# leavesnight/VIEO_SLAM

Measured on AMD Instinct MI355X. Metric: frontend+localBA frames/sec on EuRoC MH05 stereo-VIO; ATE vs ref, higher is better.
Workload: dtype u8 (extract/match) + f64 (pose optimisation)

## Files before the change

### include/vieo_hot.h

```cpp
#ifndef VIEO_HOT_H
#define VIEO_HOT_H

#include <stddef.h>
#include <stdint.h>

#ifdef __cplusplus
extern "C" {
#endif

#define VIEO_OK 0
#define VIEO_E_INVALID (-1)
#define VIEO_E_NO_DEVICE (-2)
#define VIEO_E_HIP (-3)
#define VIEO_E_CAPACITY (-4)
#define VIEO_E_EMPTY (-5)

const char* vieo_last_error(void);
int vieo_device_available(void);
int vieo_set_device(int device);
int vieo_get_device(void);
const char* vieo_version(void);

int vieo_dev_malloc(void** d_ptr, size_t bytes);
int vieo_dev_free(void* d_ptr);
// ... 582 lines not shown
                                            const int32_t* d_cam_first, int n_cams, int key_cap, int n_frames, int img_first,
                                            int img_step, const float* d_inv_sigma2, vieo_pose_obs* d_obs, int32_t* d_obs_key,
                                            void* d_frames, int frames_are_vio, void* stream);
int vieo_track_build_obs_depth_batch_device(const int32_t* d_mp_ref, const float* d_point_xyz,
                                            const float* d_point_depth, float close_depth, int p_cap,
                                            const vieo_keypoint* d_keys, const float* d_uright,
                                            const int32_t* d_counts, int key_cap, int n_frames,
                                            int img_first, int img_step, const float* d_inv_sigma2,
                                            vieo_pose_obs* d_obs, int32_t* d_obs_key, void* d_frames,
                                            int frames_are_vio, void* stream);
int vieo_track_merge_assign_rig_batch_device(const int32_t* d_assign, int32_t* d_mp_ref, const int32_t* d_counts,
                                             int key_cap, int n_frames, int img_first, int img_step, int point_offset,
                                             int reset, int query_div,
                                             const vieo_last_frame_point* d_same_point ,
                                             const int32_t* d_query_src , int q_cap, void* stream);
int vieo_track_compact_queries_batch_device(const vieo_proj_query* d_queries, const int32_t* d_nq, int q_cap, int n_frames,
                                            vieo_proj_query* d_queries_out, int32_t* d_src, int32_t* d_nq_out, void* stream);
int vieo_track_build_obs_rig_batch_device(const int32_t* d_mp_ref, const float* d_point_xyz,
                                          const float* d_point_depth, float close_depth, int p_cap,
                                          const vieo_keypoint* d_keys, const float* d_uright,
                                          const int32_t* d_counts, const int32_t* d_cam_first, int n_cams, int key_cap,
                                          int n_frames, const float* d_inv_sigma2, vieo_pose_obs* d_obs,
                                          int32_t* d_obs_key, void* d_frames, int frames_are_vio, void* stream);
int vieo_track_mark_held_batch_device(const int32_t* d_mp_ref, const int32_t* d_counts, int key_cap,
                                      int n_frames, int img_first, int img_step, uint8_t* d_held, int p_cap,
                                      void* stream);
void* vieo_orb_stream(vieo_orb* e);

int vieo_orb_tap_plane(vieo_orb* e, int image_index, int level, int which, uint8_t* h_dst,
                       int dst_stride);
int vieo_orb_tap_candidates(vieo_orb* e, int image_index, int level, int32_t* h_dst, int cap);
int vieo_orb_tap_level_keys(vieo_orb* e, int image_index, int level, vieo_keypoint* h_dst,
                            int cap);


typedef struct vieo_frustum_frame {
  float Rcrw[9], tcrw[3];
  float Ow[3];
  int32_t n_cams;
  int32_t use_distort;
  const struct vieo_camera* cams;
  float Tcr[4][12];
  float trc[4][3];
  float bounds[4][4];
  float bf;
  float log_scale_factor;
  int32_t n_levels;
  float viewing_cos_limit;
} vieo_frustum_frame;

typedef struct vieo_frustum_point {
  float Xw[3], normal[3];
  float max_distance, min_distance;
} vieo_frustum_point;

typedef struct vieo_track_info {
  float u[4], v[4], ur[4], viewcos[4];
  int32_t level[4], cam[4];
  int32_t n;
  float track_depth;
} vieo_track_info;

int vieo_is_in_frustum_batch(const vieo_frustum_frame* h_frame, const vieo_frustum_point* h_points, int n_points,
                             vieo_track_info* h_info);
int vieo_track_local_queries_device(const vieo_frustum_frame* h_frame, const vieo_vio_frame* d_frame,
                                    const vieo_vio_result* d_result, const vieo_frustum_point* d_points,
// ... 220 lines not shown
```

### vieo_slam_amd/_lib.py

```python
import ctypes
import os

_HERE = os.path.dirname(os.path.abspath(__file__))
LIB_PATH = os.environ.get("VIEO_LIB_PATH") or os.path.join(_HERE, "libvieo_hot.so")

VIEO_OK = 0
VIEO_E_INVALID, VIEO_E_NO_DEVICE, VIEO_E_HIP, VIEO_E_CAPACITY, VIEO_E_EMPTY = -1, -2, -3, -4, -5

c_p = ctypes.c_void_p
c_i = ctypes.c_int
c_f = ctypes.c_float
c_sz = ctypes.c_size_t
P = ctypes.POINTER

_SIGS = {
    "vieo_last_error": (ctypes.c_char_p, []),
    "vieo_device_available": (c_i, []),
    "vieo_set_device": (c_i, [c_i]),
    "vieo_pose_set_camera_mode": (c_i, [c_i]),
    "vieo_pose_set_replicas": (c_i, [c_i]),
    "vieo_search_for_triangulation": (c_i, [c_p, c_p, c_i, c_i, c_i, c_i, c_i, c_p, c_p, c_p]),
    "vieo_pose_set_encoder_mode": (c_i, [c_i]),
    "vieo_triangulate_new_points": (c_i, [c_p, c_p, c_p, c_p, c_i, c_f, c_i, c_i, c_p, c_p, c_p, c_p, c_p, c_p]),
    "vieo_create_new_map_points": (c_i, [c_p, c_p, c_p, c_p, c_i, c_i, c_i, c_f, c_i, c_i, c_p, c_p, c_p, c_p, c_p, c_p, c_p]),
# ... 101 lines not shown
                                                       c_p, c_i, c_p]),
    "vieo_track_mark_held_batch_device": (c_i, [c_p, c_p, c_i, c_i, c_i, c_i, c_p, c_i, c_p]),
    "vieo_track_after_pose_held_batch_device": (c_i, [c_p, c_p, c_p, c_p, c_p, c_i, c_i, c_i, c_p, c_p, c_p, c_i, c_i, c_p, c_i, c_p]),
    "vieo_track_merge_build_obs_batch_device": (c_i, [c_p, c_p, c_i, c_i, c_i, c_p, c_p, c_i, c_p, c_p, c_f, c_i, c_p, c_p, c_p, c_p, c_i,
                                                       c_i, c_i, c_i, c_i, c_p, c_p, c_p, c_p, c_i, c_p]),
    "vieo_track_local_queries_device": (c_i, [c_p, c_p, c_p, c_p, c_p, c_p, c_p, c_i, c_i, c_f, c_f, c_p, c_p, c_p, c_p, c_p]),
    "vieo_orb_stream": (c_p, [c_p]),
    "vieo_local_bundle_adjustment": (c_i, [c_p, c_p, c_i, c_p, c_i, c_p, c_i, c_p, c_p, c_p, c_p, c_p]),
    "vieo_local_bundle_adjustment_batch": (c_i, [c_i, c_p, c_p, c_p, c_p, c_p, c_p, c_p, c_p, c_p, c_p, c_p,
                                                  c_p]),
    "vieo_local_bundle_adjustment_vio": (c_i, [c_p, c_p, c_i, c_p, c_p, c_i, c_p, c_i, c_p, c_i, c_p, c_p, c_p,
                                                c_p, c_p]),
    "vieo_local_bundle_adjustment_vio_batch": (c_i, [c_i] + [c_p] * 15),
    "vieo_lba_sharded_buffer_doubles": (ctypes.c_size_t, [c_i, c_p]),
    "vieo_lba_enable_timing": (None, [c_i]),
    "vieo_lba_set_stream_priority": (c_i, [c_i]),
    "vieo_lba_kernel_classes": (c_i, []),
    "vieo_lba_kernel_class_name": (ctypes.c_char_p, [c_i]),
    "vieo_lba_kernel_times": (None, [c_p, c_p, c_p]),
    "vieo_lba_sparse_stats": (None, [c_p]),
    "vieo_rccl_available": (c_i, []),
    "vieo_rccl_unique_id": (c_i, [c_p]),
    "vieo_rccl_comm_create": (c_i, [P(c_p), c_p, c_i, c_i]),
    "vieo_rccl_comm_destroy": (c_i, [c_p]),
    "vieo_global_bundle_adjustment_vio_sharded": (c_i, [c_p, c_i, c_i, c_p, c_i, c_p, c_i, c_p, c_i, c_p, c_i, c_p,
                                                        ctypes.c_size_t, c_p, c_p, c_p, c_p, c_p]),
    "vieo_local_bundle_adjustment_vio_sharded": (c_i, [c_i] + [c_p] * 10 + [c_p, ctypes.c_size_t, c_p, c_p] +
                                                 [c_p] * 4),
    "vieo_local_bundle_adjustment_vio_sharded_stop": (c_i, [c_i] + [c_p] * 10 + [c_p, ctypes.c_size_t, c_p, c_p, c_p] +
                                                      [c_p] * 4),
    "vieo_orb_tap_plane": (c_i, [c_p, c_i, c_i, c_i, c_p, c_i]),
    "vieo_orb_tap_candidates": (c_i, [c_p, c_i, c_i, c_p, c_i]),
    "vieo_orb_tap_level_keys": (c_i, [c_p, c_i, c_i, c_p, c_i]),
    "vieo_imu_preintegrate_batch_device": (c_i, [c_p] * 7 + [c_i] + [c_p] * 4),
    "vieo_imu_preintegrate_batch_device_ex": (c_i, [c_p] * 7 + [c_i] + [c_p] * 7),
    "vieo_tracker_create": (c_i, [P(c_p), c_p]),
    "vieo_tracker_create_rig": (c_i, [P(c_p), c_p, c_p]),
    "vieo_tracker_key_capacity": (c_i, [c_p]),
    "vieo_tracker_group_capacity": (c_i, [c_p]),
    "vieo_tracker_image_buffer": (c_i, [c_p, c_i, P(c_p)]),
    "vieo_tracker_destroy": (None, [c_p]),
    "vieo_tracker_image_buffers": (c_i, [c_p, P(c_p), P(c_p)]),
    "vieo_tracker_scale_factors": (c_i, [c_p, c_p]),
    "vieo_track_frame": (c_i, [c_p, c_p, c_p]),
    "vieo_tracker_get_stats": (c_i, [c_p, c_p]),
    "vieo_tracker_reprobe": (c_i, [c_p]),
    "vieo_tracker_get_level": (c_i, [c_p, c_i, c_i, c_i, c_p, c_i]),
    "vieo_tracker_multi_create": (c_i, [P(c_p), c_p, c_i]),
    "vieo_tracker_multi_destroy": (None, [c_p]),
    "vieo_tracker_multi_image_buffer": (c_i, [c_p, c_i, c_i, P(c_p)]),
    "vieo_tracker_multi_reset_slot": (c_i, [c_p, c_i]),
    "vieo_track_frames": (c_i, [c_p, c_i, c_p, c_p, c_p]),
    "vieo_track_local_queries_slot_batch_device": (c_i, [c_p, c_p, c_sz, c_p, c_sz, c_i, c_p, c_p, c_p, c_p, c_p, c_i, c_p, c_i,
                                                         c_f, c_f, c_p, c_p, c_p, c_sz, c_p, c_p]),
}

_lib = None


class VieoError(RuntimeError):
    pass


def declared_symbols():
    return sorted(_SIGS)

# ... 55 lines not shown
```

### vieo_slam_amd/csrc/orb_extractor.hip

```cpp
#include <algorithm>
#include <cmath>
#include <type_traits>
#include <vector>

#include "../../include/vieo_orb_pattern_31.h"
#include "common.h"
#include "sincosf_exact.h"
#include "wave_ops.h"

#define QT_DEVICE
#include "quadtree.inl"

#include "orb_internal.h"

namespace vieo {

#ifndef VIEO_RESIZE_ROWS
#define VIEO_RESIZE_ROWS 32
#endif
static const int kResizeRows = VIEO_RESIZE_ROWS;
#ifndef VIEO_QT_GROUPS
#define VIEO_QT_GROUPS {1, 64}
#endif

// ... 690 lines not shown
    const unsigned oe = ((e[0] >> 16) & 0xFFu) | (((e[1] >> 16) & 0xFFu) << 8) | (((e[2] >> 16) & 0xFFu) << 16) |
                        (((e[3] >> 16) & 0xFFu) << 24);
    const unsigned oo = ((o[0] >> 16) & 0xFFu) | (((o[1] >> 16) & 0xFFu) << 8) | (((o[2] >> 16) & 0xFFu) << 16) |
                        (((o[3] >> 16) & 0xFFu) << 24);
    *(unsigned*)(dst + (size_t)gy * D.pitch + gx) = oe;
    if (gy + 1 < D.h) *(unsigned*)(dst + (size_t)(gy + 1) * D.pitch + gx) = oo;
  }
}

__device__ __forceinline__ int wave_sum(int v) { return wave_sum_i32(v); }

__device__ __forceinline__ float fast_atan2_deg(float y, float x) {
  const float p1 = 0.9997878412794807f * (float)(180 / 3.1415926535897932384626433832795);
  const float p3 = -0.3258083974640975f * (float)(180 / 3.1415926535897932384626433832795);
  const float p5 = 0.1555786518463281f * (float)(180 / 3.1415926535897932384626433832795);
  const float p7 = -0.04432655554792128f * (float)(180 / 3.1415926535897932384626433832795);
  const float eps = (float)2.2204460492503131e-16;
  const float ax = fabsf(x), ay = fabsf(y);
  float a, c, c2;
  if (ax >= ay) {
    c = ay / (ax + eps);
    c2 = c * c;
    a = (((p7 * c2 + p5) * c2 + p3) * c2 + p1) * c;
  } else {
    c = ax / (ay + eps);
    c2 = c * c;
    a = 90.f - (((p7 * c2 + p5) * c2 + p3) * c2 + p1) * c;
  }
  if (x < 0) a = 180.f - a;
  if (y < 0) a = 360.f - a;
  return a;
}

__global__ void __launch_bounds__(256)
k_desc_index(OrbParams P, const unsigned* __restrict__ sel, const int* __restrict__ sel_count,
             uint2* __restrict__ krec, int out_cap, int* __restrict__ counts) {
  const int b = blockIdx.y, g = blockIdx.x * 256 + threadIdx.x;
  int level = -1, idx = 0, total = 0;
  for (int l = 0; l < P.nlevels; l++) {
    const int n = max(sel_count[b * kMaxLevels + l], 0);
    if (level < 0 && g < total + n) {
      level = l;
      idx = g - total;
    }
    total += n;
  }
  if (g == 0) {
    counts[2 * b] = min(total, out_cap);
    counts[2 * b + 1] = 0;
  }
  if (g >= P.kp_cap) return;
  unsigned key = 0;
  if (level >= 0) key = sel[(size_t)b * P.sel_per_image + P.lv[level].sel_off + idx];
  krec[(size_t)b * P.kp_cap + g] = make_uint2(key, (unsigned)level);
}

#ifndef VIEO_DESC_KPW
#define VIEO_DESC_KPW 1
#endif
__global__ void __launch_bounds__(256)
k_describe(OrbParams P, ImgSet I, const uint2* __restrict__ krec, const int* __restrict__ pattern,
           vieo_keypoint* __restrict__ kp_out, uint8_t* __restrict__ desc_out, int out_cap,
           int groups_per_image, int n_images) {
  constexpr int KPW = VIEO_DESC_KPW;
  const int item = xcd_grouped(blockIdx.x, groups_per_image);
  const int b = item / groups_per_image;
  if (b >= n_images) return;
  const int lane = threadIdx.x & 63;
  const int wv = __builtin_amdgcn_readfirstlane((int)(threadIdx.x >> 6));
  const int g0 = ((item - b * groups_per_image) * (blockDim.x >> 6) + wv) * KPW;
  const int gmax = min(P.kp_cap, out_cap);
  if (g0 >= gmax) return;
  uint2 kr[KPW];
#pragma unroll
  for (int u = 0; u < KPW; u++) kr[u] = g0 + u < gmax ? krec[(size_t)b * P.kp_cap + g0 + u] : make_uint2(0, 0xFFFFFFFFu);
  constexpr int AP = 40, BR = 19, BP = 44;
  __shared__ __attribute__((aligned(16))) uint8_t s_patch[4][KPW][31 * AP + (2 * BR + 1) * BP];
  int pt4[4];
#pragma unroll
  for (int gq = 0; gq < 4; gq++) pt4[gq] = pattern[gq * 64 + lane];
  int cxs[KPW], cys[KPW], xas[KPW], xbs[KPW];
  unsigned va[KPW][8], vb[KPW][10];
  const int c = lane & 15, r0 = lane >> 4;
#pragma unroll
  for (int u = 0; u < KPW; u++) {
    const int level = (int)kr[u].y;
    if (level < 0) continue;
    const unsigned key = kr[u].x;
    const LevelDesc& D = P.lv[level];
    const int cx = QT_KEY_X(key) + (kEdge - 3), cy = QT_KEY_Y(key) + (kEdge - 3);
    int pitch;
    const uint8_t* img = plane_ptr(P, I, b, level, &pitch);
    const int xa = (cx - kHalfPatch) & ~3, xb = (cx - BR) & ~3;
    cxs[u] = cx, cys[u] = cy, xas[u] = xa, xbs[u] = xb;
    const uint8_t* bl0 = I.blur + (size_t)b * I.blur_img + D.boff;
    const int bp = D.pitch;
    const uint8_t* ga = img + (size_t)(cy - kHalfPatch + r0) * pitch + xa + 4 * c;
    const uint8_t* gb = bl0 + (size_t)(cy - BR + r0) * bp + xb + 4 * c;
#pragma unroll
    for (int k = 0; k < 8; k++)
      if (c < 9 && r0 + 4 * k < 31) va[u][k] = *(const unsigned*)(ga + (size_t)(4 * k) * pitch);
#pragma unroll
    for (int k = 0; k < 10; k++)
      if (c < 11 && r0 + 4 * k < 2 * BR + 1) vb[u][k] = *(const unsigned*)(gb + (size_t)(4 * k) * bp);
  }
#pragma unroll
  for (int u = 0; u < KPW; u++) {
    if ((int)kr[u].y < 0) continue;
// ... 42 lines not shown
    const float factorPI = (float)(3.1415926535897932384626433832795 / 180.f);
    float a, bsin;
    vieo_sincosf_exact(angle * factorPI, &bsin, &a);
    const uint8_t* bl = sb + BR * BP + (cx - xb);
    unsigned long long bits[4];
#pragma unroll
    for (int gq = 0; gq < 4; gq++) {
      const int pt = pt4[gq];
      const float x0 = (float)(signed char)(pt & 0xFF), y0 = (float)(signed char)((pt >> 8) & 0xFF);
      const float x1 = (float)(signed char)((pt >> 16) & 0xFF), y1 = (float)(signed char)((pt >> 24) & 0xFF);
      const int t0 = bl[__float2int_rn(x0 * bsin + y0 * a) * BP + __float2int_rn(x0 * a - y0 * bsin)];
      const int t1 = bl[__float2int_rn(x1 * bsin + y1 * a) * BP + __float2int_rn(x1 * a - y1 * bsin)];
      bits[gq] = __ballot(t0 < t1);
    }
    if (lane < 4) ((unsigned long long*)(desc_out + ((size_t)b * out_cap + g) * 32))[lane] = bits[lane];
    if (lane == 0) {
      vieo_keypoint k;
      const float fx = (float)cx, fy = (float)cy;
      k.x = level ? fx * D.scale : fx;
      k.y = level ? fy * D.scale : fy;
      k.size = (float)D.patch;
      k.angle = angle;
      k.response = (float)QT_KEY_R(key);
      k.octave = level;
      k.class_id = -1;
      kp_out[(size_t)b * out_cap + g] = k;
    }
  }
}

#ifndef VIEO_FUSED_AB
#define VIEO_FUSED_AB 0
#endif
constexpr int kFR = 18, kFRaw = kFR + 3;
constexpr int kFRawRows = 2 * kFRaw + 1, kFRawPitch = 48;
constexpr int kFHPairs = (kFRawRows + 1) / 2, kFHCols = 40;
constexpr int kFBlRows = 2 * kFR + 1, kFBlPitch = 40;
constexpr int kFWaveLds = kFRawRows * kFRawPitch + 16 + kFHPairs * kFHCols * 4;
static_assert(kFBlRows * kFBlPitch <= kFRawRows * kFRawPitch, "the blurred patch fits where the raw one was");

#ifndef VIEO_FUSED_KPW
#define VIEO_FUSED_KPW 4
#endif
static inline int fused_kpw(int n_images) { return n_images >= 32 ? VIEO_FUSED_KPW : 1; }
__global__ void __launch_bounds__(256)
k_describe_fused(OrbParams P, ImgSet I, const uint2* __restrict__ krec, const int* __restrict__ pattern,
                 vieo_keypoint* __restrict__ kp_out, uint8_t* __restrict__ desc_out, int out_cap,
                 int groups_per_image, int n_images, int KPW) {
  const int item = xcd_grouped(blockIdx.x, groups_per_image);
  const int b = item / groups_per_image;
  if (b >= n_images) return;
  const int lane = threadIdx.x & 63;
  const int wv = __builtin_amdgcn_readfirstlane((int)(threadIdx.x >> 6));
  const int g0 = ((item - b * groups_per_image) * (blockDim.x >> 6) + wv) * KPW;
  const int gmax = min(P.kp_cap, out_cap);
  if (g0 >= gmax) return;
  __shared__ __attribute__((aligned(16))) uint8_t s_all[4][kFWaveLds];
  int pt4[4];
#pragma unroll
  for (int gq = 0; gq < 4; gq++) pt4[gq] = pattern[gq * 64 + lane];
  uint8_t* s_raw = s_all[wv];
  unsigned* s_h = (unsigned*)(s_raw + kFRawRows * kFRawPitch + 16);
  constexpr int NLD = (kFRawRows + 3) / 4;
  unsigned v[NLD];
  bool interior = false;
  int sh = 0;
  const int c = lane & 15, r0 = lane >> 4;
  auto rec_of = [&](int u) { return (u < KPW && g0 + u < gmax) ? krec[(size_t)b * P.kp_cap + g0 + u] : make_uint2(0u, 0xFFFFFFFFu); };
  auto fetch = [&](const uint2 kr) {
    const int level = (int)kr.y;
    if (level < 0) return;
    const LevelDesc& D = P.lv[level];
    const int cx = QT_KEY_X(kr.x) + (kEdge - 3), cy = QT_KEY_Y(kr.x) + (kEdge - 3);
    int pitch;
    const uint8_t* img = plane_ptr(P, I, b, level, &pitch);
    const int x_lo = cx - kFRaw, y_lo = cy - kFRaw;
    const int xa = x_lo & ~3;
    sh = x_lo - xa;
    interior = x_lo >= 0 && y_lo >= 0 && cx + kFRaw < D.w && cy + kFRaw < D.h && xa + 52 <= pitch && ((pitch & 3) == 0) &&
               ((((uintptr_t)img) & 3) == 0);
    if (VIEO_FUSED_AB & 2) {
#pragma unroll
      for (int k = 0; k < NLD; k++) v[k] = kr.x + k;
      interior = false;
    } else if (interior) {
      const uint8_t* gp = img + (size_t)(y_lo + r0) * pitch + xa + 4 * c;
#pragma unroll
      for (int k = 0; k < NLD; k++) {
        v[k] = 0;
        if (c < 13 && r0 + 4 * k < kFRawRows) v[k] = *(const unsigned*)(gp + (size_t)(4 * k) * pitch);
      }
    } else {
#pragma unroll
      for (int k = 0; k < NLD; k++) {
        v[k] = 0;
        if (c < 12 && r0 + 4 * k < kFRawRows) {
          const uint8_t* row = img + (size_t)reflect101(min(max(y_lo + r0 + 4 * k, -(D.h - 1)), 2 * D.h - 2), D.h) * pitch;
#pragma unroll
          for (int jj = 0; jj < 4; jj++) {
            const int x = min(max(x_lo + 4 * c + jj, -(D.w - 1)), 2 * D.w - 2);
            v[k] |= (unsigned)row[reflect101(x, D.w)] << (8 * jj);
          }
        }
      }
    }
  };
  uint2 kr = rec_of(0);
  fetch(kr);
#pragma unroll 1
  for (int u = 0; u < KPW; u++) {
    const uint2 cur = kr;
    const int level = (int)cur.y;
    if (level < 0) break;
    const unsigned key = cur.x;
    const int g = g0 + u;
    const LevelDesc& D = P.lv[level];
    const int cx = QT_KEY_X(key) + (kEdge - 3), cy = QT_KEY_Y(key) + (kEdge - 3);
    if (interior) {
#pragma unroll
      for (int k = 0; k < NLD; k++) {
        const unsigned nxt = (unsigned)__builtin_amdgcn_update_dpp(0, (int)v[k], 0x101, 0xF, 0xF, false);
        v[k] = __builtin_amdgcn_alignbyte(nxt, v[k], sh);
      }
    }
#pragma unroll
    for (int k = 0; k < NLD; k++)
      if (c < 12 && r0 + 4 * k < kFRawRows) *(unsigned*)(s_raw + (r0 + 4 * k) * kFRawPitch + 4 * c) = v[k];
    __builtin_amdgcn_fence(__ATOMIC_ACQ_REL, "workgroup");
    __builtin_amdgcn_wave_barrier();
    kr = rec_of(u + 1);
    fetch(kr);
    {
      constexpr unsigned A0 = 18u | (34u << 8) | (48u << 16) | (56u << 24), A1 = 48u | (34u << 8) | (18u << 16);
      constexpr unsigned B0 = (18u << 8) | (34u << 16) | (48u << 24), B1 = 56u | (48u << 8) | (34u << 16) | (18u << 24);
      constexpr unsigned C0 = (18u << 16) | (34u << 24), C1 = 48u | (56u << 8) | (48u << 16) | (34u << 24), C2 = 18u;
      constexpr unsigned E0 = 18u << 24, E1 = 34u | (48u << 8) | (56u << 16) | (48u << 24), E2 = 34u | (18u << 8);
      for (int idx = lane; idx < ((VIEO_FUSED_AB & 1) ? 0 : kFHPairs * (kFHCols / 8)); idx += 64) {
        const int pr = idx / (kFHCols / 8), g8 = idx - pr * (kFHCols / 8);
        unsigned h[2][8];
#pragma unroll
        for (int q = 0; q < 2; q++) {
          const int r = min(2 * pr + q, kFRawRows - 1);
          const uint2* w = (const uint2*)(s_raw + r * kFRawPitch + 8 * g8);
          const uint2 lo = w[0], hi = w[1];
          const unsigned d0 = lo.x, d1 = lo.y, d2 = hi.x, d3 = hi.y;
#define DOT4(x, k, acc) __builtin_amdgcn_udot4(x, k, acc, false)
          h[q][0] = DOT4(d1, A1, DOT4(d0, A0, 0u));
          h[q][1] = DOT4(d1, B1, DOT4(d0, B0, 0u));
          h[q][2] = DOT4(d2, C2, DOT4(d1, C1, DOT4(d0, C0, 0u)));
          h[q][3] = DOT4(d2, E2, DOT4(d1, E1, DOT4(d0, E0, 0u)));
          h[q][4] = DOT4(d2, A1, DOT4(d1, A0, 0u));
          h[q][5] = DOT4(d2, B1, DOT4(d1, B0, 0u));
          h[q][6] = DOT4(d3, C2, DOT4(d2, C1, DOT4(d1, C0, 0u)));
          h[q][7] = DOT4(d3, E2, DOT4(d2, E1, DOT4(d1, E0, 0u)));
#undef DOT4
        }
        uint4 o0, o1;
        o0.x = h[0][0] | (h[1][0] << 16), o0.y = h[0][1] | (h[1][1] << 16);
        o0.z = h[0][2] | (h[1][2] << 16), o0.w = h[0][3] | (h[1][3] << 16);
        o1.x = h[0][4] | (h[1][4] << 16), o1.y = h[0][5] | (h[1][5] << 16);
        o1.z = h[0][6] | (h[1][6] << 16), o1.w = h[0][7] | (h[1][7] << 16);
        uint4* dst = (uint4*)(s_h + pr * kFHCols + 8 * g8);
        dst[0] = o0, dst[1] = o1;
      }
    }
    int m10 = 0, m01 = 0;
    if (lane < ((VIEO_FUSED_AB & 4) ? 1 : 62)) {
      const int vv = (lane >> 1) - kHalfPatch;
      const int d = P.umax[vv < 0 ? -vv : vv];
      const uint8_t* row = s_raw + (vv + kFRaw) * kFRawPitch + kFRaw;
      const int u0 = (lane & 1) ? 0 : -d, u1 = (lane & 1) ? d : -1;
      int sI = 0;
#pragma unroll
      for (int t = 0; t < 16; t++) {
        const int uu = u0 + t;
        if (uu <= u1) {
          const int val = row[uu];
          m10 += uu * val;
          sI += val;
        }
      }
      m01 = vv * sI;
    }
    m10 = wave_sum(m10);
    m01 = wave_sum(m01);
    const float angle = fast_atan2_deg((float)m01, (float)m10);
    __builtin_amdgcn_fence(__ATOMIC_ACQ_REL, "workgroup");
    __builtin_amdgcn_wave_barrier();
    typedef unsigned short us2 __attribute__((ext_vector_type(2)));
    uint8_t* s_bl = s_raw;
    for (int idx = lane; idx < ((VIEO_FUSED_AB & 1) ? 0 : ((kFBlRows + 1) / 2) * (kFBlPitch / 4)); idx += 64) {
      const int q = idx / (kFBlPitch / 4), c4 = (idx - q * (kFBlPitch / 4)) * 4;
      const unsigned We[4] = {18u | (34u << 16), 48u | (56u << 16), 48u | (34u << 16), 18u};
      const unsigned Wo[4] = {18u << 16, 34u | (48u << 16), 56u | (48u << 16), 34u | (18u << 16)};
      unsigned e[4] = {1u << 15, 1u << 15, 1u << 15, 1u << 15}, o[4] = {1u << 15, 1u << 15, 1u << 15, 1u << 15};
#pragma unroll
      for (int k = 0; k < 4; k++) {
        const uint4 hv = *(const uint4*)(s_h + (q + k) * kFHCols + c4);
        const unsigned vv[4] = {hv.x, hv.y, hv.z, hv.w};
#pragma unroll
        for (int jj = 0; jj < 4; jj++) {
          e[jj] = __builtin_amdgcn_udot2(__builtin_bit_cast(us2, vv[jj]), __builtin_bit_cast(us2, We[k]), e[jj], false);
          o[jj] = __builtin_amdgcn_udot2(__builtin_bit_cast(us2, vv[jj]), __builtin_bit_cast(us2, Wo[k]), o[jj], false);
        }
      }
      const unsigned oe = __builtin_amdgcn_perm(__builtin_amdgcn_perm(e[3], e[2], 0x0c0c0602u), __builtin_amdgcn_perm(e[1], e[0], 0x0c0c0602u), 0x05040100u);
      const unsigned oo = __builtin_amdgcn_perm(__builtin_amdgcn_perm(o[3], o[2], 0x0c0c0602u), __builtin_amdgcn_perm(o[1], o[0], 0x0c0c0602u), 0x05040100u);
      *(unsigned*)(s_bl + (2 * q) * kFBlPitch + c4) = oe;
      if (2 * q + 1 < kFBlRows) *(unsigned*)(s_bl + (2 * q + 1) * kFBlPitch + c4) = oo;
    }
    __builtin_amdgcn_fence(__ATOMIC_ACQ_REL, "workgroup");
    __builtin_amdgcn_wave_barrier();
    const float factorPI = (float)(3.1415926535897932384626433832795 / 180.f);
    float a, bsin;
    vieo_sincosf_exact(angle * factorPI, &bsin, &a);
// ... 305 lines not shown
      p.Htail = (unsigned)(0x80808080ull & ((1ull << (8 * (vw - 4 * (ng - 1)))) - 1ull));
      p.clear = ((vh + 2) * (vw + 2) + 15) / 16 | (vw + 2) << 16;
    }
  }
  if (P.ncells > 1) {
    int L = 1;
    while ((1 << L) < P.ncells) L++;
    e->cell_div_mul = (unsigned)((((unsigned long long)1 << (31 + L)) + P.ncells - 1) / P.ncells);
    e->cell_div_shift = L - 1;
  } else {
    e->cell_div_mul = 0, e->cell_div_shift = 0;
  }
  e->qt_lds = 16 * e->scap_max + (4 + 16 + 4 + 4 + 4) * ncap_max + 64 + (2 * 4 + 8 + 2 * 6) * ncap_max +
              ncap_max + 64;
  int rc;
#define ENS(buf, bytes)                 \
  if ((rc = (buf).ensure(bytes)) != VIEO_OK) return rc
  ENS(e->d_pyr, e->pyr_img * B);
  if (!orb_fused()) ENS(e->d_blur, e->blur_img * B);
  ENS(e->d_cells, plans.size() * sizeof(CellPlan));
  ENS(e->d_tiles, e->tiles.size() * sizeof(BlurTile));
  ENS(e->d_xtab, std::max<size_t>(xtab.size() * 2, 8));
  ENS(e->d_ytab, std::max<size_t>(ytab.size() * 2, 8));
  ENS(e->d_cell_keys, (size_t)B * P.ncells * P.cell_cap * 4);
  ENS(e->d_cell_counts, (size_t)B * P.ncells * 4);
  ENS(e->d_keys, (size_t)B * P.keys_per_image * 4);
  ENS(e->d_kslot, (size_t)B * P.keys_per_image * 2);
  ENS(e->d_kq, (size_t)B * P.keys_per_image);
  ENS(e->d_sel, (size_t)B * P.sel_per_image * 4);
  ENS(e->d_sel_count, (size_t)B * kMaxLevels * 4);
  ENS(e->d_tmp_kp, (size_t)B * P.kp_cap * sizeof(vieo_keypoint));
  ENS(e->d_tmp_desc, (size_t)B * P.kp_cap * 32);
  ENS(e->d_tmp_counts, (size_t)B * 2 * 4);
  ENS(e->d_krec, (size_t)B * P.kp_cap * 8);
#undef ENS
  VIEO_HIP_CHECK(hipMemcpyAsync(e->d_cells.p, plans.data(), plans.size() * sizeof(CellPlan),
                                hipMemcpyHostToDevice, e->stream));
  VIEO_HIP_CHECK(hipMemcpyAsync(e->d_tiles.p, e->tiles.data(), e->tiles.size() * sizeof(BlurTile),
                                hipMemcpyHostToDevice, e->stream));
  if (!xtab.empty()) {
    VIEO_HIP_CHECK(hipMemcpyAsync(e->d_xtab.p, xtab.data(), xtab.size() * 2, hipMemcpyHostToDevice,
                                  e->stream));
    VIEO_HIP_CHECK(hipMemcpyAsync(e->d_ytab.p, ytab.data(), ytab.size() * 2, hipMemcpyHostToDevice,
                                  e->stream));
  }
  VIEO_HIP_CHECK(hipStreamSynchronize(e->stream));
  if (e->qt_lds > 64 * 1024)
    VIEO_HIP_CHECK(hipFuncSetAttribute((const void*)k_quadtree,
                                       hipFuncAttributeMaxDynamicSharedMemorySize, e->qt_lds));
  if (e->qt_lds > 160 * 1024) {
    set_error("nfeatures too large for the LDS quadtree (%d bytes)", e->qt_lds);
    return VIEO_E_INVALID;
  }
  e->w = w;
  e->h = h;
  e->B = B;
  return VIEO_OK;
}

static int run_batch(vieo_orb* e, const uint8_t* d_images, int B, int w, int h, int stride,
                     size_t image_pitch, const int* lapping, vieo_keypoint* d_kp, uint8_t* d_desc,
                     int capacity, int32_t* d_counts) {
  int rc;
  if (w != e->w || h != e->h || B > e->B) {
    if ((rc = plan_geometry(e, w, h, std::max(B, (w == e->w && h == e->h) ? e->B : 0))) != VIEO_OK)
      return rc;
  }
// ... 67 lines not shown
    static const int qt_env = [] {
      const char* e = getenv("VIEO_QT_THREADS");
      const int v = e ? atoi(e) : 0;
      return v > 0 ? std::min(std::max(v / 64 * 64, 64), 1024) : 0;
    }();
    const int qt_threads = qt_env > 0 ? qt_env : (B <= 16 ? 512 : 256);
    for (size_t gi = 0; gi < n_bounds && la < P.nlevels; gi++) {
      const int lb = std::min(bounds[gi], P.nlevels);
      if (lb <= la) continue;
      int nc, sc;
      qt_caps(la, lb, &nc, &sc);
      const size_t lds = (size_t)16 * sc + (4 + 16 + 4 + 4 + 4) * nc + 64 + (2 * 4 + 8 + 2 * 6) * nc + nc + 64;
      hipLaunchKernelGGL(k_quadtree, dim3(lb - la, B), dim3(qt_threads), lds, st, P,
                         e->d_cell_keys.as<unsigned>(), e->d_cell_counts.as<int>(),
                         e->d_keys.as<unsigned>(), e->d_kslot.as<unsigned short>(),
                         e->d_kq.as<unsigned char>(), e->d_sel.as<unsigned>(), e->d_sel_count.as<int>(), nc, sc, la);
      la = lb;
    }
  }
  STAMP();
  const bool fused = orb_fused();
  if (!fused) {
    int rc_b = e->d_blur.ensure(e->blur_img * (size_t)e->B);
    if (rc_b != VIEO_OK) return rc_b;
    I.blur = e->d_blur.as<uint8_t>(), e->last_imgs = I;
    hipLaunchKernelGGL(k_blur, dim3(xcd_grid((long long)e->tiles.size() * B)), dim3(256), 0, st, P, I,
                       e->d_tiles.as<BlurTile>(), (int)e->tiles.size(), B);
  }
  STAMP();
  const int per_group = fused ? 4 * fused_kpw(B) : 4 * VIEO_DESC_KPW;
  const int ngroups = (std::min(P.kp_cap, capacity) + per_group - 1) / per_group;
  auto describe = [&](unsigned grid, vieo_keypoint* kp, uint8_t* desc, int cap, int ng) {
    if (fused)
      hipLaunchKernelGGL(k_describe_fused, dim3(grid), dim3(256), 0, st, P, I, e->d_krec.as<uint2>(), e->d_pattern.as<int>(), kp, desc,
                         cap, ng, B, fused_kpw(B));
    else
      hipLaunchKernelGGL(k_describe, dim3(grid), dim3(256), 0, st, P, I, e->d_krec.as<uint2>(), e->d_pattern.as<int>(), kp, desc, cap,
                         ng, B);
  };
  if (!lapping) {
    hipLaunchKernelGGL(k_desc_index, dim3((P.kp_cap + 255) / 256, B), dim3(256), 0, st, P, e->d_sel.as<unsigned>(),
                       e->d_sel_count.as<int>(), e->d_krec.as<uint2>(), capacity, d_counts);
    describe((unsigned)ngroups * 8 * ((B + 7) / 8), d_kp, d_desc, capacity, ngroups);
  } else {
    const int ng = (P.kp_cap + per_group - 1) / per_group;
    hipLaunchKernelGGL(k_desc_index, dim3((P.kp_cap + 255) / 256, B), dim3(256), 0, st, P, e->d_sel.as<unsigned>(),
                       e->d_sel_count.as<int>(), e->d_krec.as<uint2>(), P.kp_cap, e->d_tmp_counts.as<int>());
    describe((unsigned)ng * 8 * ((B + 7) / 8), e->d_tmp_kp.as<vieo_keypoint>(), e->d_tmp_desc.as<uint8_t>(), P.kp_cap, ng);
    hipLaunchKernelGGL(k_lapping, dim3(B), dim3(256), 0, st, e->d_tmp_kp.as<vieo_keypoint>(),
                       e->d_tmp_desc.as<uint8_t>(), P.kp_cap, d_kp, d_desc, capacity,
                       e->d_tmp_counts.as<int>(), d_counts, lapping[0], lapping[1]);
  }
  STAMP();
#undef STAMP
  if (T.on) T.steps++;
  VIEO_HIP_CHECK(hipGetLastError());
  return VIEO_OK;
}

}

extern "C" {

int vieo_orb_create(vieo_orb** out, int nfeatures, float scale_factor, int nlevels, int ini_th,
                    int min_th) {
  const char* pe = getenv("VIEO_ORB_PRIORITY");
  return vieo::orb_create_with_priority(out, nfeatures, scale_factor, nlevels, ini_th, min_th, pe && atoi(pe) > 0 ? 1 : 0);
}

}

int vieo::orb_create_with_priority(vieo_orb** out, int nfeatures, float scale_factor, int nlevels, int ini_th, int min_th,
                                   int priority) {
  if (!out || nfeatures <= 0 || nlevels <= 0 || nlevels > kMaxLevels || !(scale_factor > 1.0f)) {
    set_error("vieo_orb_create: invalid arguments");
    return VIEO_E_INVALID;
  }
  int rc = require_device();
  if (rc != VIEO_OK) return rc;
  vieo_orb* e = new vieo_orb();
// ... 22 lines not shown
  int sum = 0;
  for (int l = 0; l < nlevels - 1; l++) {
    e->feats[l] = cv_round_f(nDesired);
    sum += e->feats[l];
    nDesired *= factor;
  }
  e->feats[nlevels - 1] = std::max(nfeatures - sum, 0);
  {
    int v, v0;
    const int vmax = cv_floor_d(kHalfPatch * sqrt(2.f) / 2 + 1);
    const int vmin = cv_ceil_d(kHalfPatch * sqrt(2.f) / 2);
    const double hp2 = kHalfPatch * kHalfPatch;
    for (v = 0; v <= kHalfPatch; v++) e->umax[v] = 0;
    for (v = 0; v <= vmax; ++v) e->umax[v] = cv_round_d(sqrt(hp2 - v * v));
    for (v = kHalfPatch, v0 = 0; v >= vmin; --v) {
      while (e->umax[v0] == e->umax[v0 + 1]) ++v0;
      e->umax[v] = v0;
      ++v0;
    }
  }
  hipError_t he;
  {
    int lo = 0, hi = 0;
    if (priority > 0 && hipDeviceGetStreamPriorityRange(&lo, &hi) == hipSuccess && lo != hi)
      he = hipStreamCreateWithPriority(&e->stream, hipStreamNonBlocking, hi);
    else
      he = hipStreamCreateWithFlags(&e->stream, hipStreamNonBlocking);
  }
  if (he != hipSuccess) {
    set_error("hipStreamCreate: %s", hipGetErrorString(he));
    delete e;
    return VIEO_E_HIP;
  }
  std::vector<int> pat(256);
  for (int i = 0; i < 256; i++) {
    const signed char* p = VIEO_ORB_PATTERN_31 + i * 4;
    pat[i] = (int)((unsigned)(uint8_t)p[0] | ((unsigned)(uint8_t)p[1] << 8) |
                   ((unsigned)(uint8_t)p[2] << 16) | ((unsigned)(uint8_t)p[3] << 24));
  }
  if ((rc = e->d_pattern.ensure(1024)) != VIEO_OK) {
    delete e;
    return rc;
  }
  he = hipMemcpy(e->d_pattern.p, pat.data(), 1024, hipMemcpyHostToDevice);
  if (he != hipSuccess) {
    set_error("pattern upload: %s", hipGetErrorString(he));
    delete e;
    return VIEO_E_HIP;
  }
  for (auto& set : e->tm.ev)
    for (auto& ev : set) (void)hipEventCreate(&ev);
  *out = e;
  return VIEO_OK;
}

extern "C" {

void vieo_orb_destroy(vieo_orb* e) {
  if (!e) return;
  (void)hipStreamSynchronize(e->stream);
  DevBuf* bufs[] = {&e->d_pyr,   &e->d_blur,      &e->d_cells,    &e->d_tiles,      &e->d_xtab,
                    &e->d_ytab,  &e->d_cell_keys, &e->d_cell_counts, &e->d_keys,    &e->d_kslot,
                    &e->d_kq,    &e->d_sel,       &e->d_sel_count, &e->d_pattern,   &e->d_in,
                    &e->d_kp,    &e->d_desc,      &e->d_counts,   &e->d_tmp_kp,     &e->d_tmp_desc,
                    &e->d_tmp_counts, &e->d_krec,  &e->d_io,       &e->d_uright,     &e->d_depth,
                    &e->d_sad,   &e->g_start,     &e->g_rec,      &e->g_ang};
  for (DevBuf* b : bufs) b->release();
  e->h_in.release(), e->h_res.release(), e->h_io.release();
  for (auto& set : e->tm.ev)
    for (auto& ev : set)
      if (ev) (void)hipEventDestroy(ev);
  if (e->stream) (void)hipStreamDestroy(e->stream);
  delete e;
}

int vieo_orb_levels(const vieo_orb* e) { return e->nlevels; }
float vieo_orb_scale_factor(const vieo_orb* e) { return (float)e->scaleFactor; }
// ... 240 lines not shown
}

int vieo_orb_tap_level_keys(vieo_orb* e, int image_index, int level, vieo_keypoint* h_dst, int cap) {
  if (!e || level < 0 || level >= e->nlevels || image_index < 0 || image_index >= e->last_B)
    return VIEO_E_INVALID;
  VIEO_HIP_CHECK(hipStreamSynchronize(e->stream));
  const OrbParams& P = e->P;
  const LevelDesc& D = P.lv[level];
  int n = 0;
  VIEO_HIP_CHECK(hipMemcpy(&n, e->d_sel_count.as<int>() + image_index * kMaxLevels + level, 4,
                           hipMemcpyDeviceToHost));
  if (n < 0) {
    set_error("quadtree capacity overflow at level %d", level);
    return VIEO_E_CAPACITY;
  }
  std::vector<unsigned> keys(std::max(n, 1));
  VIEO_HIP_CHECK(hipMemcpy(keys.data(),
                           e->d_sel.as<unsigned>() + (size_t)image_index * P.sel_per_image + D.sel_off,
                           (size_t)n * 4, hipMemcpyDeviceToHost));
  for (int i = 0; i < n && i < cap; i++) {
    vieo_keypoint k;
    k.x = (float)(QT_KEY_X(keys[i]) + kEdge - 3);
    k.y = (float)(QT_KEY_Y(keys[i]) + kEdge - 3);
    k.size = (float)D.patch;
    k.angle = -1.f;
    k.response = (float)QT_KEY_R(keys[i]);
    k.octave = level;
    k.class_id = -1;
    h_dst[i] = k;
  }
  return n;
}

}
```

### vieo_slam_amd/orb_extractor.py

```python
import ctypes

import numpy as np

from . import _lib
from ._lib import c_i, c_p, check, lib

KEYPOINT_DTYPE = np.dtype([("x", "<f4"), ("y", "<f4"), ("size", "<f4"), ("angle", "<f4"),
                           ("response", "<f4"), ("octave", "<i4"), ("class_id", "<i4")])
assert KEYPOINT_DTYPE.itemsize == 28

STAGES = ("pyramid", "fast", "quadtree", "blur", "describe", "total")


class ORBextractor:

    def __init__(self, nfeatures, scaleFactor, nlevels, iniThFAST, minThFAST):
        h = c_p()
        check(lib().vieo_orb_create(ctypes.byref(h), nfeatures, scaleFactor, nlevels, iniThFAST,
                                    minThFAST), "vieo_orb_create")
        self._h = h
        self.nlevels = nlevels

    def close(self):
        if getattr(self, "_h", None):
# ... 92 lines not shown
        ms = np.zeros(len(STAGES), np.float32)
        check(lib().vieo_orb_last_stage_ms(self._h, ms.ctypes.data), "last_stage_ms")
        return dict(zip(STAGES, ms.tolist()))

    def stage_ms_all(self):
        n = lib().vieo_orb_timed_steps(self._h)
        out = []
        for back in range(n - 1, -1, -1):
            ms = np.zeros(len(STAGES), np.float32)
            check(lib().vieo_orb_stage_ms(self._h, back, ms.ctypes.data), "stage_ms")
            out.append(dict(zip(STAGES, ms.tolist())))
        return out

    def tap_blurred(self, level, image_index=0):
        w, h = self.level_size(level)
        out = np.zeros((h, w), np.uint8)
        check(lib().vieo_orb_tap_plane(self._h, image_index, level, 1, out.ctypes.data,
                                       out.strides[0]))
        return out

    def tap_candidates(self, level, image_index=0, cap=200000):
        out = np.zeros((cap, 3), np.int32)
        n = lib().vieo_orb_tap_candidates(self._h, image_index, level, out.ctypes.data, cap)
        if n < 0:
            check(n, "tap_candidates")
        return out[:n].copy()

    def tap_level_keys(self, level, image_index=0, cap=8192):
        out = np.zeros(cap, KEYPOINT_DTYPE)
        n = lib().vieo_orb_tap_level_keys(self._h, image_index, level, out.ctypes.data, cap)
        if n < 0:
            check(n, "tap_level_keys")
        return out[:n].copy()
```

Measured before the change: 60890.

## Precompute patch addressing in desc index and compute ORB moments with udot4

The per-keypoint record grows to 16 bytes and carries the precomputed patch offset, pitch, alignment shift and interior flag, so the fused describe kernel no longer recomputes addressing. Interior patch loads become unconditional using 24-bit multiplies. The intensity-centroid moment loop is replaced by packed udot4 dot products against per-lane weight tables uploaded with the pattern, and pattern registers are pinned. A debug tap for the records is also added. The cost is doubled record bandwidth and extra constant registers.

```diff
diff --git a/include/vieo_hot.h b/include/vieo_hot.h
--- a/include/vieo_hot.h
+++ b/include/vieo_hot.h
@@ -638,6 +638,7 @@
 int vieo_orb_tap_candidates(vieo_orb* e, int image_index, int level, int32_t* h_dst, int cap);
 int vieo_orb_tap_level_keys(vieo_orb* e, int image_index, int level, vieo_keypoint* h_dst,
                             int cap);
+int vieo_orb_tap_desc_records(vieo_orb* e, int image_index, uint32_t* h_dst, int cap);
 
 
 typedef struct vieo_frustum_frame {
diff --git a/vieo_slam_amd/_lib.py b/vieo_slam_amd/_lib.py
--- a/vieo_slam_amd/_lib.py
+++ b/vieo_slam_amd/_lib.py
@@ -157,6 +157,7 @@
     "vieo_orb_tap_plane": (c_i, [c_p, c_i, c_i, c_i, c_p, c_i]),
     "vieo_orb_tap_candidates": (c_i, [c_p, c_i, c_i, c_p, c_i]),
     "vieo_orb_tap_level_keys": (c_i, [c_p, c_i, c_i, c_p, c_i]),
+    "vieo_orb_tap_desc_records": (c_i, [c_p, c_i, c_p, c_i]),
     "vieo_imu_preintegrate_batch_device": (c_i, [c_p] * 7 + [c_i] + [c_p] * 4),
     "vieo_imu_preintegrate_batch_device_ex": (c_i, [c_p] * 7 + [c_i] + [c_p] * 7),
     "vieo_tracker_create": (c_i, [P(c_p), c_p]),
diff --git a/vieo_slam_amd/csrc/orb_extractor.hip b/vieo_slam_amd/csrc/orb_extractor.hip
--- a/vieo_slam_amd/csrc/orb_extractor.hip
+++ b/vieo_slam_amd/csrc/orb_extractor.hip
@@ -746,9 +746,12 @@
   return a;
 }
 
+constexpr int kFR = 18, kFRaw = kFR + 3;
+constexpr int kPatWords = 256, kAngW = kPatWords, kAngWRows = 10;
+
 __global__ void __launch_bounds__(256)
-k_desc_index(OrbParams P, const unsigned* __restrict__ sel, const int* __restrict__ sel_count,
-             uint2* __restrict__ krec, int out_cap, int* __restrict__ counts) {
+k_desc_index(OrbParams P, ImgSet I, const unsigned* __restrict__ sel, const int* __restrict__ sel_count,
+             uint4* __restrict__ krec, int out_cap, int* __restrict__ counts) {
   const int b = blockIdx.y, g = blockIdx.x * 256 + threadIdx.x;
   int level = -1, idx = 0, total = 0;
   for (int l = 0; l < P.nlevels; l++) {
@@ -764,16 +767,30 @@
     counts[2 * b + 1] = 0;
   }
   if (g >= P.kp_cap) return;
-  unsigned key = 0;
-  if (level >= 0) key = sel[(size_t)b * P.sel_per_image + P.lv[level].sel_off + idx];
-  krec[(size_t)b * P.kp_cap + g] = make_uint2(key, (unsigned)level);
+  uint4 rec = make_uint4(0u, (unsigned)level, 0u, 0u);
+  if (level >= 0) {
+    const LevelDesc& D = P.lv[level];
+    const unsigned key = sel[(size_t)b * P.sel_per_image + D.sel_off + idx];
+    const int cx = QT_KEY_X(key) + (kEdge - 3), cy = QT_KEY_Y(key) + (kEdge - 3);
+    int pitch;
+    const uint8_t* img = plane_ptr(P, I, b, level, &pitch);
+    const int x_lo = cx - kFRaw, y_lo = cy - kFRaw;
+    const int xa = x_lo & ~3;
+    const long long off = (long long)y_lo * pitch + xa + (level ? D.off : 0);
+    const bool interior = x_lo >= 0 && y_lo >= 0 && cx + kFRaw < D.w && cy + kFRaw < D.h && xa + 52 <= pitch && ((pitch & 3) == 0) &&
+                          ((((uintptr_t)img) & 3) == 0) && pitch < (1 << 24) && off < (1ll << 31);
+    rec.x = key;
+    rec.z = interior ? (unsigned)off : 0u;
+    rec.w = (interior ? (unsigned)pitch | 0x80000000u : 0u) | ((unsigned)(x_lo & 3) << 24);
+  }
+  krec[(size_t)b * P.kp_cap + g] = rec;
 }
 
 #ifndef VIEO_DESC_KPW
 #define VIEO_DESC_KPW 1
 #endif
 __global__ void __launch_bounds__(256)
-k_describe(OrbParams P, ImgSet I, const uint2* __restrict__ krec, const int* __restrict__ pattern,
+k_describe(OrbParams P, ImgSet I, const uint4* __restrict__ krec, const int* __restrict__ pattern,
            vieo_keypoint* __restrict__ kp_out, uint8_t* __restrict__ desc_out, int out_cap,
            int groups_per_image, int n_images) {
   constexpr int KPW = VIEO_DESC_KPW;
@@ -785,9 +802,9 @@
   const int g0 = ((item - b * groups_per_image) * (blockDim.x >> 6) + wv) * KPW;
   const int gmax = min(P.kp_cap, out_cap);
   if (g0 >= gmax) return;
-  uint2 kr[KPW];
-#pragma unroll
-  for (int u = 0; u < KPW; u++) kr[u] = g0 + u < gmax ? krec[(size_t)b * P.kp_cap + g0 + u] : make_uint2(0, 0xFFFFFFFFu);
+  uint4 kr[KPW];
+#pragma unroll
+  for (int u = 0; u < KPW; u++) kr[u] = g0 + u < gmax ? krec[(size_t)b * P.kp_cap + g0 + u] : make_uint4(0u, 0xFFFFFFFFu, 0u, 0u);
   constexpr int AP = 40, BR = 19, BP = 44;
   __shared__ __attribute__((aligned(16))) uint8_t s_patch[4][KPW][31 * AP + (2 * BR + 1) * BP];
   int pt4[4];
@@ -896,19 +913,21 @@
 #ifndef VIEO_FUSED_AB
 #define VIEO_FUSED_AB 0
 #endif
-constexpr int kFR = 18, kFRaw = kFR + 3;
 constexpr int kFRawRows = 2 * kFRaw + 1, kFRawPitch = 48;
 constexpr int kFHPairs = (kFRawRows + 1) / 2, kFHCols = 40;
 constexpr int kFBlRows = 2 * kFR + 1, kFBlPitch = 40;
 constexpr int kFWaveLds = kFRawRows * kFRawPitch + 16 + kFHPairs * kFHCols * 4;
 static_assert(kFBlRows * kFBlPitch <= kFRawRows * kFRawPitch, "the blurred patch fits where the raw one was");
 
+#ifndef VIEO_FUSED_PIN
+#define VIEO_FUSED_PIN 1
+#endif
 #ifndef VIEO_FUSED_KPW
 #define VIEO_FUSED_KPW 4
 #endif
 static inline int fused_kpw(int n_images) { return n_images >= 32 ? VIEO_FUSED_KPW : 1; }
 __global__ void __launch_bounds__(256)
-k_describe_fused(OrbParams P, ImgSet I, const uint2* __restrict__ krec, const int* __restrict__ pattern,
+k_describe_fused(OrbParams P, ImgSet I, const uint4* __restrict__ krec, const int* __restrict__ pattern,
                  vieo_keypoint* __restrict__ kp_out, uint8_t* __restrict__ desc_out, int out_cap,
                  int groups_per_image, int n_images, int KPW) {
   const int item = xcd_grouped(blockIdx.x, groups_per_image);
@@ -920,9 +939,6 @@
   const int gmax = min(P.kp_cap, out_cap);
   if (g0 >= gmax) return;
   __shared__ __attribute__((aligned(16))) uint8_t s_all[4][kFWaveLds];
-  int pt4[4];
-#pragma unroll
-  for (int gq = 0; gq < 4; gq++) pt4[gq] = pattern[gq * 64 + lane];
   uint8_t* s_raw = s_all[wv];
   unsigned* s_h = (unsigned*)(s_raw + kFRawRows * kFRawPitch + 16);
   constexpr int NLD = (kFRawRows + 3) / 4;
@@ -930,31 +946,37 @@
   bool interior = false;
   int sh = 0;
   const int c = lane & 15, r0 = lane >> 4;
-  auto rec_of = [&](int u) { return (u < KPW && g0 + u < gmax) ? krec[(size_t)b * P.kp_cap + g0 + u] : make_uint2(0u, 0xFFFFFFFFu); };
-  auto fetch = [&](const uint2 kr) {
+  const int vv = (lane >> 1) - kHalfPatch;
+  const unsigned* s_ang = (const unsigned*)(s_raw + (vv + kFRaw) * kFRawPitch + 4 + 16 * (lane & 1));
+  const uint8_t* const base0 = I.img0 + (size_t)b * I.img_pitch;
+  const uint8_t* const basel = I.pyr + (size_t)b * I.pyr_img;
+  const unsigned cc = 4 * min(c, 12);
+  auto rec_of = [&](int u) { return (u < KPW && g0 + u < gmax) ? krec[(size_t)b * P.kp_cap + g0 + u] : make_uint4(0u, 0xFFFFFFFFu, 0u, 0u); };
+  auto fetch = [&](const uint4 kr) {
     const int level = (int)kr.y;
     if (level < 0) return;
-    const LevelDesc& D = P.lv[level];
-    const int cx = QT_KEY_X(kr.x) + (kEdge - 3), cy = QT_KEY_Y(kr.x) + (kEdge - 3);
-    int pitch;
-    const uint8_t* img = plane_ptr(P, I, b, level, &pitch);
-    const int x_lo = cx - kFRaw, y_lo = cy - kFRaw;
-    const int xa = x_lo & ~3;
-    sh = x_lo - xa;
-    interior = x_lo >= 0 && y_lo >= 0 && cx + kFRaw < D.w && cy + kFRaw < D.h && xa + 52 <= pitch && ((pitch & 3) == 0) &&
-               ((((uintptr_t)img) & 3) == 0);
+    sh = (int)(kr.w >> 24) & 3;
+    interior = (int)kr.w < 0;
     if (VIEO_FUSED_AB & 2) {
 #pragma unroll
       for (int k = 0; k < NLD; k++) v[k] = kr.x + k;
       interior = false;
     } else if (interior) {
-      const uint8_t* gp = img + (size_t)(y_lo + r0) * pitch + xa + 4 * c;
+      const int pitch = (int)(kr.w & 0xFFFFFFu);
+      const uint8_t* rowp = (level ? basel : base0) + (int)kr.z;
+      const unsigned vo = (unsigned)__mul24(r0, pitch) + cc;
+      const unsigned vl = (unsigned)__mul24(min(r0, kFRawRows - 1 - 4 * (NLD - 1)), pitch) + cc;
 #pragma unroll
       for (int k = 0; k < NLD; k++) {
-        v[k] = 0;
-        if (c < 13 && r0 + 4 * k < kFRawRows) v[k] = *(const unsigned*)(gp + (size_t)(4 * k) * pitch);
+        v[k] = *(const unsigned*)(rowp + (k < NLD - 1 ? vo : vl));
+        rowp += 4 * pitch;
       }
     } else {
+      const LevelDesc& D = P.lv[level];
+      const int cx = QT_KEY_X(kr.x) + (kEdge - 3), cy = QT_KEY_Y(kr.x) + (kEdge - 3);
+      int pitch;
+      const uint8_t* img = plane_ptr(P, I, b, level, &pitch);
+      const int x_lo = cx - kFRaw, y_lo = cy - kFRaw;
 #pragma unroll
       for (int k = 0; k < NLD; k++) {
         v[k] = 0;
@@ -969,11 +991,23 @@
       }
     }
   };
-  uint2 kr = rec_of(0);
+  uint4 kr = rec_of(0);
   fetch(kr);
+  int pt4[4];
+#pragma unroll
+  for (int gq = 0; gq < 4; gq++) pt4[gq] = pattern[gq * 64 + lane];
+  unsigned wu[5], wm[5];
+#pragma unroll
+  for (int j = 0; j < 5; j++) wu[j] = (unsigned)pattern[kAngW + j * 64 + lane], wm[j] = (unsigned)pattern[kAngW + (5 + j) * 64 + lane];
+#if VIEO_FUSED_PIN
+#pragma unroll
+  for (int gq = 0; gq < 4; gq++) asm volatile("" : "+v"(pt4[gq]));
+#pragma unroll
+  for (int j = 0; j < 5; j++) asm volatile("" : "+v"(wu[j]), "+v"(wm[j]));
+#endif
 #pragma unroll 1
   for (int u = 0; u < KPW; u++) {
-    const uint2 cur = kr;
+    const uint4 cur = kr;
     const int level = (int)cur.y;
     if (level < 0) break;
     const unsigned key = cur.x;
@@ -983,7 +1017,7 @@
     if (interior) {
 #pragma unroll
       for (int k = 0; k < NLD; k++) {
-        const unsigned nxt = (unsigned)__builtin_amdgcn_update_dpp(0, (int)v[k], 0x101, 0xF, 0xF, false);
+        const unsigned nxt = (unsigned)__builtin_amdgcn_update_dpp(0, (int)v[k], 0x101, 0xF, 0xF, true);
         v[k] = __builtin_amdgcn_alignbyte(nxt, v[k], sh);
       }
     }
@@ -1028,23 +1062,20 @@
         dst[0] = o0, dst[1] = o1;
       }
     }
-    int m10 = 0, m01 = 0;
-    if (lane < ((VIEO_FUSED_AB & 4) ? 1 : 62)) {
-      const int vv = (lane >> 1) - kHalfPatch;
-      const int d = P.umax[vv < 0 ? -vv : vv];
-      const uint8_t* row = s_raw + (vv + kFRaw) * kFRawPitch + kFRaw;
-      const int u0 = (lane & 1) ? 0 : -d, u1 = (lane & 1) ? d : -1;
-      int sI = 0;
-#pragma unroll
-      for (int t = 0; t < 16; t++) {
-        const int uu = u0 + t;
-        if (uu <= u1) {
-          const int val = row[uu];
-          m10 += uu * val;
-          sI += val;
-        }
-      }
-      m01 = vv * sI;
+    int m10, m01;
+    {
+      unsigned px[5];
+#pragma unroll
+      for (int j = 0; j < 5; j++) px[j] = s_ang[j];
+      unsigned A = 0, S = 0;
+#pragma unroll
+      for (int j = 0; j < 5; j++) {
+        A = __builtin_amdgcn_udot4(px[j], wu[j], A, false);
+        S = __builtin_amdgcn_udot4(px[j], wm[j], S, false);
+      }
+      if ((VIEO_FUSED_AB & 4) && lane) A = S = 0;
+      m10 = (int)A - 16 * (int)S;
+      m01 = __mul24(vv, (int)S);
     }
     m10 = wave_sum(m10);
     m01 = wave_sum(m01);
@@ -1416,7 +1447,7 @@
   ENS(e->d_tmp_kp, (size_t)B * P.kp_cap * sizeof(vieo_keypoint));
   ENS(e->d_tmp_desc, (size_t)B * P.kp_cap * 32);
   ENS(e->d_tmp_counts, (size_t)B * 2 * 4);
-  ENS(e->d_krec, (size_t)B * P.kp_cap * 8);
+  ENS(e->d_krec, (size_t)B * P.kp_cap * 16);
 #undef ENS
   VIEO_HIP_CHECK(hipMemcpyAsync(e->d_cells.p, plans.data(), plans.size() * sizeof(CellPlan),
                                 hipMemcpyHostToDevice, e->stream));
@@ -1550,20 +1581,20 @@
   const int ngroups = (std::min(P.kp_cap, capacity) + per_group - 1) / per_group;
   auto describe = [&](unsigned grid, vieo_keypoint* kp, uint8_t* desc, int cap, int ng) {
     if (fused)
-      hipLaunchKernelGGL(k_describe_fused, dim3(grid), dim3(256), 0, st, P, I, e->d_krec.as<uint2>(), e->d_pattern.as<int>(), kp, desc,
+      hipLaunchKernelGGL(k_describe_fused, dim3(grid), dim3(256), 0, st, P, I, e->d_krec.as<uint4>(), e->d_pattern.as<int>(), kp, desc,
                          cap, ng, B, fused_kpw(B));
     else
-      hipLaunchKernelGGL(k_describe, dim3(grid), dim3(256), 0, st, P, I, e->d_krec.as<uint2>(), e->d_pattern.as<int>(), kp, desc, cap,
+      hipLaunchKernelGGL(k_describe, dim3(grid), dim3(256), 0, st, P, I, e->d_krec.as<uint4>(), e->d_pattern.as<int>(), kp, desc, cap,
                          ng, B);
   };
   if (!lapping) {
-    hipLaunchKernelGGL(k_desc_index, dim3((P.kp_cap + 255) / 256, B), dim3(256), 0, st, P, e->d_sel.as<unsigned>(),
-                       e->d_sel_count.as<int>(), e->d_krec.as<uint2>(), capacity, d_counts);
+    hipLaunchKernelGGL(k_desc_index, dim3((P.kp_cap + 255) / 256, B), dim3(256), 0, st, P, I, e->d_sel.as<unsigned>(),
+                       e->d_sel_count.as<int>(), e->d_krec.as<uint4>(), capacity, d_counts);
     describe((unsigned)ngroups * 8 * ((B + 7) / 8), d_kp, d_desc, capacity, ngroups);
   } else {
     const int ng = (P.kp_cap + per_group - 1) / per_group;
-    hipLaunchKernelGGL(k_desc_index, dim3((P.kp_cap + 255) / 256, B), dim3(256), 0, st, P, e->d_sel.as<unsigned>(),
-                       e->d_sel_count.as<int>(), e->d_krec.as<uint2>(), P.kp_cap, e->d_tmp_counts.as<int>());
+    hipLaunchKernelGGL(k_desc_index, dim3((P.kp_cap + 255) / 256, B), dim3(256), 0, st, P, I, e->d_sel.as<unsigned>(),
+                       e->d_sel_count.as<int>(), e->d_krec.as<uint4>(), P.kp_cap, e->d_tmp_counts.as<int>());
     describe((unsigned)ng * 8 * ((B + 7) / 8), e->d_tmp_kp.as<vieo_keypoint>(), e->d_tmp_desc.as<uint8_t>(), P.kp_cap, ng);
     hipLaunchKernelGGL(k_lapping, dim3(B), dim3(256), 0, st, e->d_tmp_kp.as<vieo_keypoint>(),
                        e->d_tmp_desc.as<uint8_t>(), P.kp_cap, d_kp, d_desc, capacity,
@@ -1652,17 +1683,29 @@
     delete e;
     return VIEO_E_HIP;
   }
-  std::vector<int> pat(256);
+  std::vector<int> pat(kPatWords);
   for (int i = 0; i < 256; i++) {
     const signed char* p = VIEO_ORB_PATTERN_31 + i * 4;
     pat[i] = (int)((unsigned)(uint8_t)p[0] | ((unsigned)(uint8_t)p[1] << 8) |
                    ((unsigned)(uint8_t)p[2] << 16) | ((unsigned)(uint8_t)p[3] << 24));
   }
-  if ((rc = e->d_pattern.ensure(1024)) != VIEO_OK) {
+  pat.resize(kAngW + kAngWRows * 64, 0);
+  for (int lane = 0; lane < 62; lane++) {
+    const int v = (lane >> 1) - kHalfPatch, d = e->umax[v < 0 ? -v : v], odd = lane & 1;
+    for (int j = 0; j < 5; j++)
+      for (int k = 0; k < 4; k++) {
+        const int u = (odd ? -1 : -17) + 4 * j + k;
+        if (odd ? (u >= 0 && u <= d) : (u >= -d && u <= -1)) {
+          pat[kAngW + j * 64 + lane] |= (u + 16) << (8 * k);
+          pat[kAngW + (5 + j) * 64 + lane] |= 1 << (8 * k);
+        }
+      }
+  }
+  if ((rc = e->d_pattern.ensure(pat.size() * 4)) != VIEO_OK) {
     delete e;
     return rc;
   }
-  he = hipMemcpy(e->d_pattern.p, pat.data(), 1024, hipMemcpyHostToDevice);
+  he = hipMemcpy(e->d_pattern.p, pat.data(), pat.size() * 4, hipMemcpyHostToDevice);
   if (he != hipSuccess) {
     set_error("pattern upload: %s", hipGetErrorString(he));
     delete e;
@@ -1969,4 +2012,18 @@
   return n;
 }
 
-}
+int vieo_orb_tap_desc_records(vieo_orb* e, int image_index, uint32_t* h_dst, int cap) {
+  if (!e || !h_dst || cap < 0 || image_index < 0 || image_index >= e->last_B) return VIEO_E_INVALID;
+  VIEO_HIP_CHECK(hipStreamSynchronize(e->stream));
+  const OrbParams& P = e->P;
+  std::vector<int> cnt(kMaxLevels);
+  VIEO_HIP_CHECK(hipMemcpy(cnt.data(), e->d_sel_count.as<int>() + image_index * kMaxLevels, kMaxLevels * 4, hipMemcpyDeviceToHost));
+  int n = 0;
+  for (int l = 0; l < P.nlevels; l++) n += std::max(cnt[l], 0);
+  n = std::min(std::min(n, P.kp_cap), cap);
+  if (n > 0)
+    VIEO_HIP_CHECK(hipMemcpy(h_dst, e->d_krec.as<uint4>() + (size_t)image_index * P.kp_cap, (size_t)n * 16, hipMemcpyDeviceToHost));
+  return n;
+}
+
+}
diff --git a/vieo_slam_amd/orb_extractor.py b/vieo_slam_amd/orb_extractor.py
--- a/vieo_slam_amd/orb_extractor.py
+++ b/vieo_slam_amd/orb_extractor.py
@@ -148,3 +148,10 @@
         if n < 0:
             check(n, "tap_level_keys")
         return out[:n].copy()
+
+    def tap_desc_records(self, image_index=0, cap=8192):
+        out = np.zeros((cap, 4), np.uint32)
+        n = lib().vieo_orb_tap_desc_records(self._h, image_index, out.ctypes.data, cap)
+        if n < 0:
+            check(n, "tap_desc_records")
+        return out[:n].copy()
```

Measured after the change: 61630, median of 6. +1.2%, better.
